# petuum/adaptdl

Hardware: AMD Instinct MI355X
Metric: goodput (samples/s x stat-eff), ResNet-18 CIFAR adaptive-BS (higher is better)
Workload: dtype bf16; 1 GPU; model=resnet18-cifar, global_batch=4096, atomic_bsz=1024, accum_steps=3, init_batch=128, max_batch=4096, parallelism=dp1

## Files before the change

adaptdl_amd/ops/hip/bindings.cpp:

```cpp

#include <torch/extension.h>
#include <ATen/hip/HIPContext.h>
#include <hip/hip_runtime.h>

#include <cmath>

#include "kernels.h"

namespace {

void check_f32(const torch::Tensor& t, const char* name) {
    TORCH_CHECK(t.is_cuda(), name, " must be a GPU tensor");
    TORCH_CHECK(t.scalar_type() == torch::kFloat32, name, " must be float32");
    TORCH_CHECK(t.is_contiguous(), name, " must be contiguous");
}

void check_out(const torch::Tensor& out) {
    TORCH_CHECK(out.is_cuda(), "out must be a GPU tensor");
    TORCH_CHECK(out.scalar_type() == torch::kFloat64, "out must be float64");
}

hipStream_t stream() {
    return at::hip::getCurrentHIPStream().stream();
}
// ... 124 lines not shown
    float bias1 = (float)(1.0 - std::pow(beta1, (double)step));
    float bias2 = (float)(1.0 - std::pow(beta2, (double)step));
    launch_fused_adamw(p.data_ptr<float>(), g.data_ptr<float>(),
                       m.data_ptr<float>(), v.data_ptr<float>(), n,
                       (float)lr, (float)beta1, (float)beta2, (float)eps,
                       (float)weight_decay, bias1, bias2, (int)adam_mode,
                       stream());
}

StatDtype check_lp_pair(const torch::Tensor& p, const torch::Tensor& g) {
    const StatDtype dtype = check_stat_in(p, "p");
    check_stat_in(g, "g");
    TORCH_CHECK(dtype != STAT_F32,
                "p must be bfloat16 or float16 (float32 parameters take "
                "fused_sgd / fused_adamw)");
    TORCH_CHECK(g.scalar_type() == p.scalar_type(), "p/g dtype mismatch");
    TORCH_CHECK(g.numel() == p.numel(), "p/g size mismatch");
    return dtype;
}

void check_f32_n(const torch::Tensor& t, long n, const char* name) {
    check_f32(t, name);
    TORCH_CHECK(t.numel() == n, name, " size mismatch");
}

void fused_sgd_mw(torch::Tensor p, torch::Tensor g, torch::Tensor w,
                  torch::Tensor m, double lr, double momentum,
                  double weight_decay, double dampening, bool nesterov) {
    const StatDtype dtype = check_lp_pair(p, g);
    long n = p.numel();
    check_f32_n(w, n, "master");
    bool has_m = momentum != 0.0;
    if (has_m) check_f32_n(m, n, "momentum_buf");
    if (n == 0) return;
    launch_fused_sgd_mw(dtype, p.data_ptr(), g.data_ptr(),
                        w.data_ptr<float>(),
                        has_m ? m.data_ptr<float>() : nullptr, n, (float)lr,
                        (float)momentum, (float)weight_decay,
                        (float)dampening, (int)nesterov, (int)has_m,
                        stream());
}

void fused_adamw_mw(torch::Tensor p, torch::Tensor g, torch::Tensor w,
                    torch::Tensor m, torch::Tensor v, double lr,
                    double beta1, double beta2, double eps,
                    double weight_decay, long step, bool adam_mode) {
    const StatDtype dtype = check_lp_pair(p, g);
    long n = p.numel();
    check_f32_n(w, n, "master");
    check_f32_n(m, n, "m"); check_f32_n(v, n, "v");
    if (n == 0) return;
    float bias1 = (float)(1.0 - std::pow(beta1, (double)step));
    float bias2 = (float)(1.0 - std::pow(beta2, (double)step));
    launch_fused_adamw_mw(dtype, p.data_ptr(), g.data_ptr(),
                          w.data_ptr<float>(), m.data_ptr<float>(),
                          v.data_ptr<float>(), n, (float)lr, (float)beta1,
                          (float)beta2, (float)eps, (float)weight_decay,
                          bias1, bias2, (int)adam_mode, stream());
}


void check_bn_x(const torch::Tensor& t, const char* name) {
    TORCH_CHECK(t.is_cuda(), name, " must be a GPU tensor");
    TORCH_CHECK(t.scalar_type() == torch::kBFloat16, name,
                " must be bfloat16");
    TORCH_CHECK(t.dim() == 4, name, " must be 4-D NCHW-shaped");
    TORCH_CHECK(t.is_contiguous(at::MemoryFormat::ChannelsLast), name,
                " must be channels_last");
}

void check_vecf(const torch::Tensor& t, long n, const char* name) {
    TORCH_CHECK(t.is_cuda() && t.scalar_type() == torch::kFloat32 &&
                t.is_contiguous() && t.numel() == n,
                name, " must be a contiguous fp32 GPU tensor of size ", n);
}

long bn_ws_rows(long m, long c) {
    TORCH_CHECK(c >= 8 && c % 8 == 0 && c / 8 <= 256,
                "bn_num_rblocks requires C % 8 == 0 and 8 <= C <= 2048, "
                "got C=", c);
    return bn_num_rblocks(m, (int)c);
}

void bn_fwd(torch::Tensor x, torch::Tensor z, torch::Tensor y,
            torch::Tensor gamma, torch::Tensor beta,
            torch::Tensor running_mean, torch::Tensor running_var,
            double momentum, double eps, bool train, bool relu,
            torch::Tensor ws, torch::Tensor sums,
            torch::Tensor save_mean, torch::Tensor save_rstd,
            torch::Tensor scale, torch::Tensor shift) {
    check_bn_x(x, "x"); check_bn_x(y, "y");
    const unsigned short* zp = nullptr;
    if (z.defined() && z.numel() > 0) {
        check_bn_x(z, "z");
        TORCH_CHECK(z.sizes() == x.sizes(), "residual shape mismatch");
        zp = (const unsigned short*)z.data_ptr();
    }
    const long c = x.size(1);
    const long m = x.numel() / c;
    TORCH_CHECK(c % 8 == 0 && c / 8 <= 256,
                "bn_fwd requires C % 8 == 0 and C <= 2048, got C=", c);
    check_vecf(gamma, c, "gamma"); check_vecf(beta, c, "beta");
    if (train)
        check_vecf(ws, 2 * c * bn_num_rblocks(m, (int)c), "ws");
    check_vecf(sums, 2 * c, "sums");
    check_vecf(save_mean, c, "save_mean");
    check_vecf(save_rstd, c, "save_rstd");
    check_vecf(scale, c, "scale"); check_vecf(shift, c, "shift");
    float* rm = nullptr;
    float* rv = nullptr;
    if (running_mean.defined() && running_mean.numel() > 0) {
        check_vecf(running_mean, c, "running_mean");
        check_vecf(running_var, c, "running_var");
        rm = running_mean.data_ptr<float>();
        rv = running_var.data_ptr<float>();
    } else {
        TORCH_CHECK(train, "eval-mode bn_fwd requires running statistics");
    }
    launch_bn_fwd((const unsigned short*)x.data_ptr(), zp,
                  (unsigned short*)y.data_ptr(), m, (int)c,
                  gamma.data_ptr<float>(), beta.data_ptr<float>(), rm, rv,
                  (float)momentum, (float)eps, (int)train, (int)relu,
                  train ? ws.data_ptr<float>() : nullptr,
                  sums.data_ptr<float>(), save_mean.data_ptr<float>(),
                  save_rstd.data_ptr<float>(), scale.data_ptr<float>(),
                  shift.data_ptr<float>(), stream());
}

void bn_bwd(torch::Tensor x, torch::Tensor z, torch::Tensor dy,
            torch::Tensor dx, torch::Tensor dz,
            torch::Tensor gamma, torch::Tensor save_mean,
            torch::Tensor save_rstd, torch::Tensor scale,
            torch::Tensor shift, bool train, bool relu, torch::Tensor ws,
            torch::Tensor sums, torch::Tensor dgamma, torch::Tensor dbeta,
            torch::Tensor pqr) {
    check_bn_x(x, "x"); check_bn_x(dy, "dy"); check_bn_x(dx, "dx");
    const unsigned short* zp = nullptr;
    unsigned short* dzp = nullptr;
    if (z.defined() && z.numel() > 0) {
        check_bn_x(z, "z"); check_bn_x(dz, "dz");
        TORCH_CHECK(z.sizes() == x.sizes(), "residual shape mismatch");
        zp = (const unsigned short*)z.data_ptr();
        dzp = (unsigned short*)dz.data_ptr();
    }
    const long c = x.size(1);
    const long m = x.numel() / c;
    check_vecf(gamma, c, "gamma");
    check_vecf(save_mean, c, "save_mean");
    check_vecf(save_rstd, c, "save_rstd");
    check_vecf(scale, c, "scale"); check_vecf(shift, c, "shift");
    check_vecf(ws, 2 * c * bn_num_rblocks(m, (int)c), "ws");
    check_vecf(sums, 2 * c, "sums");
    check_vecf(dgamma, c, "dgamma"); check_vecf(dbeta, c, "dbeta");
    check_vecf(pqr, 3 * c, "pqr");
    launch_bn_bwd((const unsigned short*)x.data_ptr(), zp,
                  (const unsigned short*)dy.data_ptr(),
                  (unsigned short*)dx.data_ptr(), dzp, m, (int)c,
                  gamma.data_ptr<float>(), save_mean.data_ptr<float>(),
                  save_rstd.data_ptr<float>(), scale.data_ptr<float>(),
                  shift.data_ptr<float>(), (int)train, (int)relu,
                  ws.data_ptr<float>(), sums.data_ptr<float>(),
                  dgamma.data_ptr<float>(), dbeta.data_ptr<float>(),
                  pqr.data_ptr<float>(), stream());
}


bool conv_wrw_ok(long N, long H, long W, long C, long K) {
    return conv3x3_wrw_supported((int)H, (int)W, (int)C, (int)K) != 0;
}

long conv_wrw_nsplit(long N, long H, long W, long C, long K) {
    return conv3x3_wrw_nsplit((int)N, (int)H, (int)W, (int)C, (int)K);
}

void conv_wrw(torch::Tensor x, torch::Tensor dy, torch::Tensor ws,
              torch::Tensor dw) {
    check_bn_x(x, "x"); check_bn_x(dy, "dy");
    const long N = x.size(0), C = x.size(1), H = x.size(2), W = x.size(3);
    const long K = dy.size(1);
    TORCH_CHECK(dy.size(0) == N && dy.size(2) == H && dy.size(3) == W,
                "dy shape mismatch");
    TORCH_CHECK(conv_wrw_ok(N, H, W, C, K), "unsupported wrw shape");
    TORCH_CHECK(dw.is_cuda() && dw.scalar_type() == torch::kFloat32 &&
                dw.is_contiguous(at::MemoryFormat::ChannelsLast) &&
                dw.size(0) == K && dw.size(1) == C && dw.size(2) == 3 &&
                dw.size(3) == 3, "dw must be (K,C,3,3) channels_last f32");
    const long nsplit = conv_wrw_nsplit(N, H, W, C, K);
    check_vecf(ws, nsplit * K * 9 * C, "ws");
    launch_conv3x3_wrw((const unsigned short*)x.data_ptr(),
                       (const unsigned short*)dy.data_ptr(),
                       ws.data_ptr<float>(), dw.data_ptr<float>(),
                       (int)N, (int)H, (int)W, (int)C, (int)K, stream());
}

bool conv_mm_ok(long N, long H, long W, long C, long K) {
    return conv3x3_mm_supported((int)H, (int)W, (int)C, (int)K) != 0;
}

void conv_mm(torch::Tensor x, torch::Tensor w, torch::Tensor y) {
    check_bn_x(x, "x"); check_bn_x(y, "y");
    const long N = x.size(0), C = x.size(1), H = x.size(2),
        Wd = x.size(3);
    const long K = y.size(1);
    TORCH_CHECK(y.size(0) == N && y.size(2) == H && y.size(3) == Wd,
                "y shape mismatch");
    TORCH_CHECK(w.is_cuda() && w.scalar_type() == torch::kBFloat16 &&
                w.is_contiguous(at::MemoryFormat::ChannelsLast) &&
                w.size(0) == K && w.size(1) == C && w.size(2) == 3 &&
                w.size(3) == 3, "w must be (K,C,3,3) channels_last bf16");
    TORCH_CHECK(conv_mm_ok(N, H, Wd, C, K), "unsupported conv_mm shape");
    launch_conv3x3_mm((const unsigned short*)x.data_ptr(),
                      (const unsigned short*)w.data_ptr(),
                      (unsigned short*)y.data_ptr(),
                      (int)N, (int)H, (int)Wd, (int)C, (int)K, stream());
}

bool conv_s2_bwd_ok(long N, long Ho, long Wo, long K, long C) {
    (void)N;
    return conv3x3_s2_bwd_supported((int)Ho, (int)Wo, (int)K, (int)C)
        != 0;
}

void conv_s2_bwd(torch::Tensor dy, torch::Tensor wt, torch::Tensor dx) {
    check_bn_x(dy, "dy"); check_bn_x(dx, "dx");
    const long N = dy.size(0), K = dy.size(1), Ho = dy.size(2),
        Wo = dy.size(3);
    const long C = dx.size(1);
    TORCH_CHECK(dx.size(0) == N && dx.size(2) == 2 * Ho &&
                dx.size(3) == 2 * Wo, "dx shape mismatch");
    TORCH_CHECK(wt.is_cuda() && wt.scalar_type() == torch::kBFloat16 &&
                wt.is_contiguous() && wt.size(0) == C &&
                wt.size(1) == 3 && wt.size(2) == 3 && wt.size(3) == K,
                "wt must be (C,3,3,K) contiguous bf16");
    TORCH_CHECK(conv_s2_bwd_ok(N, Ho, Wo, K, C),
                "unsupported s2 bwd-data shape");
    launch_conv3x3_s2_bwd((const unsigned short*)dy.data_ptr(),
                          (const unsigned short*)wt.data_ptr(),
                          (unsigned short*)dx.data_ptr(),
                          (int)N, (int)Ho, (int)Wo, (int)K, (int)C,
                          stream());
}

bool conv_s2_fwd_ok(long N, long H, long W, long C, long K) {
    (void)N;
    return conv3x3_s2_fwd_supported((int)H, (int)W, (int)C, (int)K) != 0;
}
// ... 130 lines not shown
```

adaptdl_amd/ops/hip/bn_kernels.hip:

```cpp

#include <hip/hip_runtime.h>
#include <hip/hip_bf16.h>

#include "kernels.h"

#define WAVE 64
#define BLOCK 256
#define MAX_RBLOCKS 1024
#define MAX_BLOCKS 2048
#define VEC 8

typedef unsigned short ushort_t;

union Vec8 {
    float4 f4;
    ushort_t u[VEC];
};

__device__ __forceinline__ float b2f(ushort_t h) {
    union { float f; unsigned u; } c;
    c.u = ((unsigned)h) << 16;
    return c.f;
}

__device__ __forceinline__ ushort_t f2b(float f) {
    __hip_bfloat16 h = __float2bfloat16(f);
    return *reinterpret_cast<ushort_t*>(&h);
}

__device__ __forceinline__ void rg_tree_reduce(
        float (&s)[VEC], float* lds, int slots, int rpb, int rg) {
    int p2 = 1;
    while (p2 * 2 <= rpb) p2 *= 2;
    #pragma unroll
    for (int k = 0; k < VEC; ++k) lds[threadIdx.x * VEC + k] = s[k];
    __syncthreads();
    if (rg < p2 && rg + p2 < rpb) {
        #pragma unroll
        for (int k = 0; k < VEC; ++k)
            s[k] += lds[(threadIdx.x + p2 * slots) * VEC + k];
    }
    for (int r = p2 / 2; r > 0; r >>= 1) {
        if (rg < p2) {
            #pragma unroll
            for (int k = 0; k < VEC; ++k) lds[threadIdx.x * VEC + k] = s[k];
        }
        __syncthreads();
        if (rg < r) {
            #pragma unroll
            for (int k = 0; k < VEC; ++k)
                s[k] += lds[(threadIdx.x + r * slots) * VEC + k];
        }
        __syncthreads();
    }
}

extern "C" __global__ __launch_bounds__(BLOCK) void k_bn_fwd_reduce(
        const ushort_t* __restrict__ x, long m, int c, int nb,
        float* __restrict__ ws) {
    const int slots = c / VEC;
    const int rpb = BLOCK / slots > 0 ? BLOCK / slots : 1;
    const int slot = threadIdx.x % slots;
    const int rg = threadIdx.x / slots;
    __shared__ float lds[BLOCK * VEC];

    float s[VEC], s2[VEC];
    #pragma unroll
    for (int k = 0; k < VEC; ++k) { s[k] = 0.f; s2[k] = 0.f; }

    if (rg < rpb) {
        const ushort_t* base = x + (size_t)slot * VEC;
        for (long row = (long)blockIdx.x * rpb + rg; row < m;
                row += (long)gridDim.x * rpb) {
            Vec8 v;
            v.f4 = *reinterpret_cast<const float4*>(base + (size_t)row * c);
            #pragma unroll
            for (int k = 0; k < VEC; ++k) {
                float f = b2f(v.u[k]);
                s[k] += f;
                s2[k] = fmaf(f, f, s2[k]);
            }
        }
    }
    rg_tree_reduce(s, lds, slots, rpb, rg);
    if (rg == 0) {
        #pragma unroll
        for (int k = 0; k < VEC; ++k)
            ws[(size_t)(slot * VEC + k) * nb + blockIdx.x] = s[k];
    }
    __syncthreads();
    rg_tree_reduce(s2, lds, slots, rpb, rg);
    if (rg == 0) {
        #pragma unroll
        for (int k = 0; k < VEC; ++k)
            ws[(size_t)(c + slot * VEC + k) * nb + blockIdx.x] = s2[k];
    }
}

extern "C" __global__ __launch_bounds__(BLOCK) void k_bn_reduce_ws(
        const float* __restrict__ ws, int nb, float* __restrict__ out) {
    __shared__ float lds[BLOCK];
    const float* row = ws + (size_t)blockIdx.x * nb;
    float s = 0.f;
    for (int i = threadIdx.x; i < nb; i += BLOCK) s += row[i];
    #pragma unroll
    for (int off = WAVE / 2; off > 0; off >>= 1)
        s += __shfl_down(s, off, WAVE);
    const int lane = threadIdx.x & (WAVE - 1);
    const int wid = threadIdx.x / WAVE;
    if (lane == 0) lds[wid] = s;
    __syncthreads();
    if (threadIdx.x == 0) {
        float t = 0.f;
        #pragma unroll
        for (int i = 0; i < BLOCK / WAVE; ++i) t += lds[i];
        out[blockIdx.x] = t;
    }
}

extern "C" __global__ void k_bn_fwd_finalize(
        const float* __restrict__ sums, long m, int c,
        const float* __restrict__ gamma, const float* __restrict__ beta,
        float* __restrict__ running_mean, float* __restrict__ running_var,
        float momentum, float eps,
        float* __restrict__ save_mean, float* __restrict__ save_rstd,
        float* __restrict__ scale, float* __restrict__ shift) {
    int i = blockIdx.x * blockDim.x + threadIdx.x;
    if (i >= c) return;
    float inv_m = 1.0f / (float)m;
    float mean = sums[i] * inv_m;
    float var = sums[c + i] * inv_m - mean * mean;
    var = var > 0.f ? var : 0.f;
    float rstd = rsqrtf(var + eps);
    save_mean[i] = mean;
    save_rstd[i] = rstd;
    float sc = gamma[i] * rstd;
    scale[i] = sc;
    shift[i] = beta[i] - mean * sc;
    if (running_mean != nullptr) {
        float unbiased = m > 1 ? var * (float)m / (float)(m - 1) : var;
        running_mean[i] += momentum * (mean - running_mean[i]);
        running_var[i] += momentum * (unbiased - running_var[i]);
    }
}

extern "C" __global__ void k_bn_eval_finalize(
        int c, const float* __restrict__ gamma,
        const float* __restrict__ beta,
        const float* __restrict__ running_mean,
        const float* __restrict__ running_var, float eps,
        float* __restrict__ save_mean, float* __restrict__ save_rstd,
        float* __restrict__ scale, float* __restrict__ shift) {
    int i = blockIdx.x * blockDim.x + threadIdx.x;
    if (i >= c) return;
    float mean = running_mean[i];
    float rstd = rsqrtf(running_var[i] + eps);
    save_mean[i] = mean;
    save_rstd[i] = rstd;
    float sc = gamma[i] * rstd;
    scale[i] = sc;
    shift[i] = beta[i] - mean * sc;
}

extern "C" __global__ __launch_bounds__(BLOCK) void k_bn_fwd_apply(
        const ushort_t* __restrict__ x, const ushort_t* __restrict__ z,
        ushort_t* __restrict__ y, long m, int c,
        const float* __restrict__ scale,
        const float* __restrict__ shift, int relu) {
    const int slots = c / VEC;
    const int rpb = BLOCK / slots > 0 ? BLOCK / slots : 1;
    const int slot = threadIdx.x % slots;
    const int rg = threadIdx.x / slots;
    if (rg >= rpb) return;
    float sc[VEC], sh[VEC];
    #pragma unroll
    for (int k = 0; k < VEC; ++k) {
        sc[k] = scale[slot * VEC + k];
        sh[k] = shift[slot * VEC + k];
    }
    const ushort_t* xb = x + (size_t)slot * VEC;
    const ushort_t* zb = z ? z + (size_t)slot * VEC : nullptr;
    ushort_t* yb = y + (size_t)slot * VEC;
    for (long row = (long)blockIdx.x * rpb + rg; row < m;
            row += (long)gridDim.x * rpb) {
        Vec8 in, vz, out;
        in.f4 = *reinterpret_cast<const float4*>(xb + (size_t)row * c);
        if (zb)
            vz.f4 = *reinterpret_cast<const float4*>(zb + (size_t)row * c);
        #pragma unroll
        for (int k = 0; k < VEC; ++k) {
            float f = fmaf(b2f(in.u[k]), sc[k], sh[k]);
            if (zb) f += b2f(vz.u[k]);
            if (relu) f = f > 0.f ? f : 0.f;
            out.u[k] = f2b(f);
        }
        *reinterpret_cast<float4*>(yb + (size_t)row * c) = out.f4;
    }
}

extern "C" __global__ __launch_bounds__(BLOCK) void k_bn_bwd_reduce(
        const ushort_t* __restrict__ x, const ushort_t* __restrict__ z,
        const ushort_t* __restrict__ dy,
        long m, int c, int nb, const float* __restrict__ mean,
        const float* __restrict__ rstd, const float* __restrict__ scale,
        const float* __restrict__ shift, int relu,
        float* __restrict__ ws) {
    const int slots = c / VEC;
    const int rpb = BLOCK / slots > 0 ? BLOCK / slots : 1;
    const int slot = threadIdx.x % slots;
    const int rg = threadIdx.x / slots;
    __shared__ float lds[BLOCK * VEC];

    float sg[VEC], sgx[VEC];
    float mn[VEC], rs[VEC], sc[VEC], sh[VEC];
    #pragma unroll
    for (int k = 0; k < VEC; ++k) {
        sg[k] = 0.f; sgx[k] = 0.f;
        mn[k] = mean[slot * VEC + k];
        rs[k] = rstd[slot * VEC + k];
        sc[k] = scale[slot * VEC + k];
        sh[k] = shift[slot * VEC + k];
    }
    if (rg < rpb) {
        const ushort_t* xb = x + (size_t)slot * VEC;
        const ushort_t* zb = z ? z + (size_t)slot * VEC : nullptr;
        const ushort_t* db = dy + (size_t)slot * VEC;
        for (long row = (long)blockIdx.x * rpb + rg; row < m;
                row += (long)gridDim.x * rpb) {
            Vec8 vx, vz, vd;
            vx.f4 = *reinterpret_cast<const float4*>(xb + (size_t)row * c);
            if (zb)
                vz.f4 = *reinterpret_cast<const float4*>(
                    zb + (size_t)row * c);
            vd.f4 = *reinterpret_cast<const float4*>(db + (size_t)row * c);
            #pragma unroll
            for (int k = 0; k < VEC; ++k) {
                float fx = b2f(vx.u[k]);
                float g = b2f(vd.u[k]);
                if (relu) {
                    float pre = fmaf(fx, sc[k], sh[k]);
                    if (zb) pre += b2f(vz.u[k]);
                    if (pre <= 0.f) g = 0.f;
                }
                sg[k] += g;
                sgx[k] = fmaf(g, (fx - mn[k]) * rs[k], sgx[k]);
            }
        }
    }
    rg_tree_reduce(sg, lds, slots, rpb, rg);
    if (rg == 0) {
        #pragma unroll
        for (int k = 0; k < VEC; ++k)
            ws[(size_t)(slot * VEC + k) * nb + blockIdx.x] = sg[k];
    }
    __syncthreads();
    rg_tree_reduce(sgx, lds, slots, rpb, rg);
    if (rg == 0) {
        #pragma unroll
        for (int k = 0; k < VEC; ++k)
            ws[(size_t)(c + slot * VEC + k) * nb + blockIdx.x] = sgx[k];
    }
}

extern "C" __global__ void k_bn_bwd_finalize(
        const float* __restrict__ sums, long m, int c,
        const float* __restrict__ gamma, const float* __restrict__ mean,
        const float* __restrict__ rstd, int train,
        float* __restrict__ dgamma, float* __restrict__ dbeta,
        float* __restrict__ pqr) {
    int i = blockIdx.x * blockDim.x + threadIdx.x;
    if (i >= c) return;
    float sum_g = sums[i];
    float sum_gx = sums[c + i];
    dbeta[i] = sum_g;
    dgamma[i] = sum_gx;
    float p = gamma[i] * rstd[i];
    float q = 0.f, r = 0.f;
    if (train) {
        float inv_m = 1.0f / (float)m;
        q = p * (sum_gx * inv_m) * rstd[i];
        r = -p * (sum_g * inv_m) + q * mean[i];
    }
    pqr[i] = p;
    pqr[c + i] = q;
    pqr[2 * c + i] = r;
}

extern "C" __global__ __launch_bounds__(BLOCK) void k_bn_bwd_apply(
        const ushort_t* __restrict__ x, const ushort_t* __restrict__ z,
        const ushort_t* __restrict__ dy,
        ushort_t* __restrict__ dx, ushort_t* __restrict__ dz, long m,
        int c, const float* __restrict__ scale,
        const float* __restrict__ shift,
        const float* __restrict__ pqr, int relu) {
    const int slots = c / VEC;
    const int rpb = BLOCK / slots > 0 ? BLOCK / slots : 1;
    const int slot = threadIdx.x % slots;
    const int rg = threadIdx.x / slots;
    if (rg >= rpb) return;
    float sc[VEC], sh[VEC], cp[VEC], cq[VEC], cr[VEC];
    #pragma unroll
    for (int k = 0; k < VEC; ++k) {
        sc[k] = scale[slot * VEC + k];
        sh[k] = shift[slot * VEC + k];
        cp[k] = pqr[slot * VEC + k];
        cq[k] = pqr[c + slot * VEC + k];
        cr[k] = pqr[2 * c + slot * VEC + k];
    }
    const ushort_t* xb = x + (size_t)slot * VEC;
    const ushort_t* zb = z ? z + (size_t)slot * VEC : nullptr;
    const ushort_t* db = dy + (size_t)slot * VEC;
    ushort_t* ob = dx + (size_t)slot * VEC;
    ushort_t* zo = dz ? dz + (size_t)slot * VEC : nullptr;
    for (long row = (long)blockIdx.x * rpb + rg; row < m;
            row += (long)gridDim.x * rpb) {
        Vec8 vx, vz, vd, out, outz;
        vx.f4 = *reinterpret_cast<const float4*>(xb + (size_t)row * c);
        if (zb)
            vz.f4 = *reinterpret_cast<const float4*>(zb + (size_t)row * c);
        vd.f4 = *reinterpret_cast<const float4*>(db + (size_t)row * c);
        #pragma unroll
        for (int k = 0; k < VEC; ++k) {
            float fx = b2f(vx.u[k]);
            float g = b2f(vd.u[k]);
            if (relu) {
                float pre = fmaf(fx, sc[k], sh[k]);
                if (zb) pre += b2f(vz.u[k]);
                if (pre <= 0.f) g = 0.f;
            }
            if (zo) outz.u[k] = f2b(g);
            out.u[k] = f2b(fmaf(cp[k], g, fmaf(-cq[k], fx, cr[k])));
        }
        *reinterpret_cast<float4*>(ob + (size_t)row * c) = out.f4;
        if (zo)
            *reinterpret_cast<float4*>(zo + (size_t)row * c) = outz.f4;
    }
}


static inline unsigned bn_grid(long work_items, int per_block, long cap) {
    long blocks = (work_items + per_block - 1) / per_block;
    if (blocks > cap) blocks = cap;
    if (blocks < 1) blocks = 1;
    return (unsigned)blocks;
}

static inline int bn_rows_per_block(int c) {
    const int slots = c / VEC;
    return BLOCK / slots > 0 ? BLOCK / slots : 1;
}

extern "C" long bn_num_rblocks(long m, int c) {
    return bn_grid(m, bn_rows_per_block(c), MAX_RBLOCKS);
}

extern "C" void launch_bn_fwd(
        const ushort_t* x, const ushort_t* z, ushort_t* y, long m, int c,
        const float* gamma, const float* beta, float* running_mean,
        float* running_var, float momentum, float eps, int train, int relu,
        float* ws, float* sums, float* save_mean, float* save_rstd,
        float* scale, float* shift, hipStream_t s) {
    const int rpb = bn_rows_per_block(c);
    if (train) {
        const unsigned nb = (unsigned)bn_num_rblocks(m, c);
        hipLaunchKernelGGL(k_bn_fwd_reduce, dim3(nb), dim3(BLOCK), 0, s,
                           x, m, c, (int)nb, ws);
        hipLaunchKernelGGL(k_bn_reduce_ws, dim3(2 * c), dim3(BLOCK), 0, s,
                           ws, (int)nb, sums);
        hipLaunchKernelGGL(k_bn_fwd_finalize,
                           dim3((c + BLOCK - 1) / BLOCK), dim3(BLOCK), 0, s,
                           sums, m, c, gamma, beta, running_mean,
                           running_var, momentum, eps, save_mean, save_rstd,
                           scale, shift);
    } else {
        hipLaunchKernelGGL(k_bn_eval_finalize,
                           dim3((c + BLOCK - 1) / BLOCK), dim3(BLOCK), 0, s,
                           c, gamma, beta, running_mean, running_var, eps,
                           save_mean, save_rstd, scale, shift);
    }
    hipLaunchKernelGGL(k_bn_fwd_apply, dim3(bn_grid(m, rpb, MAX_BLOCKS)),
                       dim3(BLOCK), 0, s, x, z, y, m, c, scale, shift,
                       relu);
}

extern "C" void launch_bn_bwd(
        const ushort_t* x, const ushort_t* z, const ushort_t* dy,
        ushort_t* dx, ushort_t* dz, long m, int c,
        const float* gamma, const float* save_mean, const float* save_rstd,
        const float* scale, const float* shift, int train, int relu,
        float* ws, float* sums, float* dgamma, float* dbeta, float* pqr,
        hipStream_t s) {
    const int rpb = bn_rows_per_block(c);
    const unsigned nb = (unsigned)bn_num_rblocks(m, c);
    hipLaunchKernelGGL(k_bn_bwd_reduce, dim3(nb), dim3(BLOCK), 0, s,
                       x, z, dy, m, c, (int)nb, save_mean, save_rstd,
                       scale, shift, relu, ws);
    hipLaunchKernelGGL(k_bn_reduce_ws, dim3(2 * c), dim3(BLOCK), 0, s,
                       ws, (int)nb, sums);
    hipLaunchKernelGGL(k_bn_bwd_finalize, dim3((c + BLOCK - 1) / BLOCK),
                       dim3(BLOCK), 0, s, sums, m, c, gamma, save_mean,
                       save_rstd, train, dgamma, dbeta, pqr);
    hipLaunchKernelGGL(k_bn_bwd_apply, dim3(bn_grid(m, rpb, MAX_BLOCKS)),
                       dim3(BLOCK), 0, s, x, z, dy, dx, dz, m, c, scale,
                       shift, pqr, relu);
}
```

adaptdl_amd/ops/hip/kernels.h:

```cpp

#pragma once

#include <hip/hip_runtime_api.h>

extern "C" {

enum StatDtype { STAT_F32 = 0, STAT_BF16 = 1, STAT_FP16 = 2 };


void launch_sqsum(StatDtype dtype, const void* x, long n, double* out,
                  hipStream_t s);
void launch_scale_sqsum(StatDtype dtype, void* x, long n, float scale,
                        double* out, hipStream_t s);
void launch_sqsum_diff_update(StatDtype dtype, const void* cur, void* prev,
                              long n, double* out, hipStream_t s);
void launch_sqsum_avg(StatDtype dtype, const void* cur, const void* prev,
                      long n, double* out, hipStream_t s);
void launch_precond_sqsum(const float* g, const float* v, long n,
                          float inv_corr_sqrt, float eps, double* out,
                          hipStream_t s);
void launch_precond_sqsum_dev(const float* g, const float* v, long n,
                              const float* pc, double* out, hipStream_t s);
void launch_fused_sgd(float* p, const float* g, float* m, long n, float lr,
                      float momentum, float weight_decay, float dampening,
                      int nesterov, int has_momentum, hipStream_t s);
void launch_fused_adamw(float* p, const float* g, float* m, float* v,
                        long n, float lr, float beta1, float beta2,
                        float eps, float weight_decay, float bias1,
                        float bias2, int adam_mode, hipStream_t s);

void launch_precond_sqsum_mw(StatDtype dtype, const void* g,
                             const float* v, long n, float inv_corr_sqrt,
                             float eps, double* out, hipStream_t s);
void launch_precond_sqsum_dev_mw(StatDtype dtype, const void* g,
                                 const float* v, long n, const float* pc,
                                 double* out, hipStream_t s);
void launch_fused_sgd_mw(StatDtype dtype, void* p, const void* g,
                         float* w, float* m, long n, float lr,
                         float momentum, float weight_decay,
                         float dampening, int nesterov, int has_momentum,
                         hipStream_t s);
void launch_fused_adamw_mw(StatDtype dtype, void* p, const void* g,
                           float* w, float* m, float* v, long n, float lr,
                           float beta1, float beta2, float eps,
                           float weight_decay, float bias1, float bias2,
                           int adam_mode, hipStream_t s);


long bn_num_rblocks(long m, int c);
void launch_bn_fwd(const unsigned short* x, const unsigned short* z,
                   unsigned short* y, long m, int c, const float* gamma,
                   const float* beta, float* running_mean,
                   float* running_var, float momentum, float eps,
                   int train, int relu, float* ws, float* sums,
                   float* save_mean, float* save_rstd, float* scale,
                   float* shift, hipStream_t s);
void launch_bn_bwd(const unsigned short* x, const unsigned short* z,
                   const unsigned short* dy, unsigned short* dx,
                   unsigned short* dz, long m, int c, const float* gamma,
                   const float* save_mean, const float* save_rstd,
                   const float* scale, const float* shift, int train,
                   int relu, float* ws, float* sums, float* dgamma,
                   float* dbeta, float* pqr, hipStream_t s);


int conv3x3_wrw_params(int H, int W, int* P, int* Wp);
int conv3x3_wrw_supported(int H, int W, int C, int K);
int conv3x3_wrw_nsplit(int N, int H, int W, int C, int K);
void launch_conv3x3_wrw(const unsigned short* x, const unsigned short* dy,
                        float* ws, float* dw, int N, int H, int W, int C,
                        int K, hipStream_t s);
int conv3x3_mm_supported(int H, int W, int C, int K);
void launch_conv3x3_mm(const unsigned short* x, const unsigned short* w,
                       unsigned short* y, int N, int H, int W, int C,
                       int K, hipStream_t s);
int conv3x3_s2_fwd_supported(int H, int W, int C, int K);
void launch_conv3x3_s2_fwd(const unsigned short* x,
                           const unsigned short* w, unsigned short* y,
                           int N, int H, int W, int C, int K,
                           hipStream_t s);
int conv3x3_s2_bwd_supported(int Ho, int Wo, int K, int C);
void launch_conv3x3_s2_bwd(const unsigned short* dy,
                           const unsigned short* wt, unsigned short* dx,
                           int N, int Ho, int Wo, int K, int C,
                           hipStream_t s);
int conv3x3_s2_wrw_supported(int Ho, int Wo, int C, int K);
int conv3x3_s2_wrw_nsplit(int N, int Ho, int Wo, int C, int K);
void launch_conv3x3_s2_wrw(const unsigned short* x,
                           const unsigned short* dy, float* ws, float* dw,
                           int N, int Ho, int Wo, int C, int K,
                           hipStream_t s);
int conv3x3_s2_bwd_w8b_supported(int Ho, int Wo, int K, int C);
void launch_conv3x3_s2_bwd_w8b(const unsigned short* dy,
                               const unsigned short* wt,
                               unsigned short* dx, int N, int Ho, int K,
                               int C, hipStream_t s);

}
```

adaptdl_amd/torch/layers.py:

```python

import os

import torch
import torch.nn as nn
import torch.nn.functional as F

from adaptdl_amd import ops


def _hip_bn_ok(x):
    c = x.shape[1] if x.dim() == 4 else 0
    return (x.is_cuda and x.dtype == torch.bfloat16 and x.dim() == 4 and
            c % 8 == 0 and c // 8 <= 256 and
            x.is_contiguous(memory_format=torch.channels_last) and
            ops.has_extension())


class _FusedBNFunction(torch.autograd.Function):
    @staticmethod
    def forward(ctx, x, z, weight, bias, running_mean, running_var,
                training, momentum, eps, relu):
        ext = ops._load_extension()
        y = torch.empty_like(x)
        c = x.shape[1]
        m = x.numel() // c
        opt = dict(dtype=torch.float32, device=x.device)
        ws = torch.empty(2 * c * ext.bn_num_rblocks(m, c), **opt) \
            if training else torch.empty(0, **opt)
        sums = torch.empty(2 * c, **opt)
        save_mean = torch.empty(c, **opt)
        save_rstd = torch.empty(c, **opt)
        scale = torch.empty(c, **opt)
        shift = torch.empty(c, **opt)
        none = torch.empty(0, **opt)
        znone = torch.empty(0, dtype=x.dtype, device=x.device)
        ext.bn_fwd(x, z if z is not None else znone, y, weight, bias,
                   running_mean if running_mean is not None else none,
                   running_var if running_var is not None else none,
                   float(momentum), float(eps), bool(training), bool(relu),
                   ws, sums, save_mean, save_rstd, scale, shift)
        ctx.save_for_backward(x, z if z is not None else znone, weight,
                              save_mean, save_rstd, scale, shift)
        ctx.bn_train = bool(training)
        ctx.bn_relu = bool(relu)
        ctx.bn_has_z = z is not None
        return y

    @staticmethod
    def backward(ctx, dy):
        ext = ops._load_extension()
        x, z, weight, save_mean, save_rstd, scale, shift = \
            ctx.saved_tensors
        dy = dy.contiguous(memory_format=torch.channels_last)
        dx = torch.empty_like(x)
        dz = torch.empty_like(x) if ctx.bn_has_z else \
            torch.empty(0, dtype=x.dtype, device=x.device)
        c = x.shape[1]
        m = x.numel() // c
        opt = dict(dtype=torch.float32, device=x.device)
        ws = torch.empty(2 * c * ext.bn_num_rblocks(m, c), **opt)
        sums = torch.empty(2 * c, **opt)
        dgamma = torch.empty(c, **opt)
        dbeta = torch.empty(c, **opt)
        pqr = torch.empty(3 * c, **opt)
        ext.bn_bwd(x, z, dy, dx, dz, weight, save_mean, save_rstd, scale,
                   shift, ctx.bn_train, ctx.bn_relu, ws, sums, dgamma,
                   dbeta, pqr)
        return (dx, dz if ctx.bn_has_z else None, dgamma, dbeta) + \
            (None,) * 6


class FusedBatchNormAct2d(nn.BatchNorm2d):

    def __init__(self, num_features, eps=1e-5, momentum=0.1, affine=True,
                 track_running_stats=True, relu=False):
        super().__init__(num_features, eps=eps, momentum=momentum,
                         affine=affine,
                         track_running_stats=track_running_stats)
        self.relu = relu

    def forward(self, x, residual=None):
        use_batch_stats = self.training or not self.track_running_stats
        if _hip_bn_ok(x) and self.affine and \
                (residual is None or
                 (residual.dtype == x.dtype and residual.is_contiguous(
                     memory_format=torch.channels_last))):
            if self.training and self.track_running_stats and \
                    self.num_batches_tracked is not None:
                self.num_batches_tracked.add_(1)
            momentum = self.momentum if self.momentum is not None else 0.0
            return _FusedBNFunction.apply(
                x, residual, self.weight, self.bias, self.running_mean,
                self.running_var, use_batch_stats, momentum, self.eps,
                self.relu)
        y = super().forward(x)
        if residual is not None:
            y = y + residual
        return F.relu(y) if self.relu else y


class _FusedConvFunction(torch.autograd.Function):

    @staticmethod
    def forward(ctx, x, weight, wb, stride, padding, dilation, groups):
        ext = ops._load_extension()
        n, c, h, w = x.shape
        k = wb.shape[0]
        if os.getenv("ADAPTDL_EXPERIMENTAL_CONV_MM") == "1" \
                and ext.conv_mm_ok(n, h, w, c, k):
            y = torch.empty(n, k, h, w, dtype=x.dtype, device=x.device) \
                .contiguous(memory_format=torch.channels_last)
            ext.conv_mm(x, wb, y)
        else:
            y = torch.nn.functional.conv2d(x, wb, None, stride, padding,
                                           dilation, groups)
        ctx.save_for_backward(x, wb)
        ctx.conv_args = (stride, padding, dilation, groups)
        return y

    @staticmethod
    def backward(ctx, dy):
        ext = ops._load_extension()
        x, wb = ctx.saved_tensors
        stride, padding, dilation, groups = ctx.conv_args
        dy = dy.contiguous(memory_format=torch.channels_last)
        dx = None
        if ctx.needs_input_grad[0]:
            n, c, h, w = x.shape
            k = wb.shape[0]
            if os.getenv("ADAPTDL_EXPERIMENTAL_CONV_MM") == "1" \
                    and ext.conv_mm_ok(n, h, w, k, c):
                wt = wb.flip(2, 3).permute(1, 0, 2, 3) \
                    .contiguous(memory_format=torch.channels_last)
                dx = torch.empty_like(x)
                ext.conv_mm(dy, wt, dx)
            else:
                dx = torch.ops.aten.convolution_backward(
                    dy, x, wb, None, stride, padding, dilation, False,
                    [0, 0], groups, [True, False, False])[0]
        n, c, h, w = x.shape
        k = dy.shape[1]
        nsplit = ext.conv_wrw_nsplit(n, h, w, c, k)
        ws = torch.empty(nsplit * k * 9 * c, dtype=torch.float32,
                         device=x.device)
        dw = torch.empty(k, c, 3, 3, dtype=torch.float32,
                         device=x.device) \
            .contiguous(memory_format=torch.channels_last)
        ext.conv_wrw(x, dy, ws, dw)
        return dx, dw, None, None, None, None, None


class _S2ConvFunction(torch.autograd.Function):

    @staticmethod
    def forward(ctx, x, weight, stride, padding, dilation, groups):
        wb = weight.detach().to(torch.bfloat16) \
            .contiguous(memory_format=torch.channels_last)
        y = torch.nn.functional.conv2d(x, wb, None, stride, padding,
                                       dilation, groups)
        ctx.save_for_backward(x, wb)
        ctx.conv_args = (stride, padding, dilation, groups)
        return y

    @staticmethod
    def backward(ctx, dy):
        ext = ops._load_extension()
        x, wb = ctx.saved_tensors
        stride, padding, dilation, groups = ctx.conv_args
        dy = dy.contiguous(memory_format=torch.channels_last)
        dx = dw = None
        if ctx.needs_input_grad[0]:
            wt = wb.permute(1, 2, 3, 0).contiguous()
            dx = torch.empty_like(x)
            n2, k2, ho2, wo2 = dy.shape
            if os.getenv("ADAPTDL_S2_W8B") == "1" and wo2 == 8 \
                    and ext.conv_s2_bwd_w8b_ok(n2, ho2, wo2, k2,
                                               x.shape[1]):
# ... 130 lines not shown
```

Baseline: 22210 goodput-samples/s.

## Fuse BN workspace reduce into finalize tail and save ReLU mask for residual BN

Merges the separate workspace row-reduction and finalize kernels into one per-channel tail kernel in both BN forward and backward, removing a launch and the intermediate sums buffer. The num_batches_tracked increment moves into that kernel, dropping a separate PyTorch add op. For ReLU+residual BN, the forward pass writes a 1-bit-per-element mask so backward can skip re-reading the residual and recomputing the pre-activation. This costs an extra uint8 write in forward, and the residual is no longer kept for backward.

Result: faster. 22880 goodput-samples/s, median of 6 (+3.0%).

```diff
diff --git a/adaptdl_amd/ops/hip/bindings.cpp b/adaptdl_amd/ops/hip/bindings.cpp
--- a/adaptdl_amd/ops/hip/bindings.cpp
+++ b/adaptdl_amd/ops/hip/bindings.cpp
@@ -230,14 +230,25 @@
     return bn_num_rblocks(m, (int)c);
 }
 
+unsigned char* bn_mask_ptr(const torch::Tensor& mask, long m, long c) {
+    if (!mask.defined() || mask.numel() == 0) return nullptr;
+    TORCH_CHECK(mask.is_cuda() && mask.scalar_type() == torch::kUInt8 &&
+                mask.is_contiguous() && mask.numel() == m * (c / 8),
+                "mask must be a contiguous uint8 GPU tensor of size ",
+                m * (c / 8));
+    return mask.data_ptr<unsigned char>();
+}
+
 void bn_fwd(torch::Tensor x, torch::Tensor z, torch::Tensor y,
             torch::Tensor gamma, torch::Tensor beta,
             torch::Tensor running_mean, torch::Tensor running_var,
             double momentum, double eps, bool train, bool relu,
-            torch::Tensor ws, torch::Tensor sums,
+            torch::Tensor ws,
             torch::Tensor save_mean, torch::Tensor save_rstd,
-            torch::Tensor scale, torch::Tensor shift) {
+            torch::Tensor scale, torch::Tensor shift,
+            torch::Tensor mask, torch::Tensor num_batches_tracked) {
     check_bn_x(x, "x"); check_bn_x(y, "y");
+    TORCH_CHECK(y.sizes() == x.sizes(), "output shape mismatch");
     const unsigned short* zp = nullptr;
     if (z.defined() && z.numel() > 0) {
         check_bn_x(z, "z");
@@ -251,7 +262,6 @@
     check_vecf(gamma, c, "gamma"); check_vecf(beta, c, "beta");
     if (train)
         check_vecf(ws, 2 * c * bn_num_rblocks(m, (int)c), "ws");
-    check_vecf(sums, 2 * c, "sums");
     check_vecf(save_mean, c, "save_mean");
     check_vecf(save_rstd, c, "save_rstd");
     check_vecf(scale, c, "scale"); check_vecf(shift, c, "shift");
@@ -265,14 +275,25 @@
     } else {
         TORCH_CHECK(train, "eval-mode bn_fwd requires running statistics");
     }
+    unsigned char* mp = bn_mask_ptr(mask, m, c);
+    TORCH_CHECK(mp == nullptr || (relu && zp != nullptr),
+                "a ReLU mask is stored only with relu and a residual");
+    long long* nbt = nullptr;
+    if (num_batches_tracked.defined() && num_batches_tracked.numel() > 0) {
+        TORCH_CHECK(num_batches_tracked.is_cuda() &&
+                    num_batches_tracked.scalar_type() == torch::kInt64 &&
+                    num_batches_tracked.numel() == 1,
+                    "num_batches_tracked must be an int64 GPU scalar");
+        nbt = (long long*)num_batches_tracked.data_ptr<int64_t>();
+    }
     launch_bn_fwd((const unsigned short*)x.data_ptr(), zp,
                   (unsigned short*)y.data_ptr(), m, (int)c,
                   gamma.data_ptr<float>(), beta.data_ptr<float>(), rm, rv,
                   (float)momentum, (float)eps, (int)train, (int)relu,
                   train ? ws.data_ptr<float>() : nullptr,
-                  sums.data_ptr<float>(), save_mean.data_ptr<float>(),
+                  save_mean.data_ptr<float>(),
                   save_rstd.data_ptr<float>(), scale.data_ptr<float>(),
-                  shift.data_ptr<float>(), stream());
+                  shift.data_ptr<float>(), mp, nbt, stream());
 }
 
 void bn_bwd(torch::Tensor x, torch::Tensor z, torch::Tensor dy,
@@ -280,25 +301,36 @@
             torch::Tensor gamma, torch::Tensor save_mean,
             torch::Tensor save_rstd, torch::Tensor scale,
             torch::Tensor shift, bool train, bool relu, torch::Tensor ws,
-            torch::Tensor sums, torch::Tensor dgamma, torch::Tensor dbeta,
-            torch::Tensor pqr) {
+            torch::Tensor dgamma, torch::Tensor dbeta,
+            torch::Tensor pqr, torch::Tensor mask) {
     check_bn_x(x, "x"); check_bn_x(dy, "dy"); check_bn_x(dx, "dx");
+    TORCH_CHECK(dy.sizes() == x.sizes() && dx.sizes() == x.sizes(),
+                "gradient shape mismatch");
+    const long c = x.size(1);
+    const long m = x.numel() / c;
+    TORCH_CHECK(c % 8 == 0 && c / 8 <= 256,
+                "bn_bwd requires C % 8 == 0 and C <= 2048, got C=", c);
     const unsigned short* zp = nullptr;
     unsigned short* dzp = nullptr;
+    const unsigned char* mp = bn_mask_ptr(mask, m, c);
     if (z.defined() && z.numel() > 0) {
-        check_bn_x(z, "z"); check_bn_x(dz, "dz");
+        check_bn_x(z, "z");
         TORCH_CHECK(z.sizes() == x.sizes(), "residual shape mismatch");
         zp = (const unsigned short*)z.data_ptr();
+    }
+    if (dz.defined() && dz.numel() > 0) {
+        check_bn_x(dz, "dz");
+        TORCH_CHECK(dz.sizes() == x.sizes(), "residual shape mismatch");
+        TORCH_CHECK(zp != nullptr || mp != nullptr,
+                    "dz requires the residual or its saved ReLU mask");
         dzp = (unsigned short*)dz.data_ptr();
     }
-    const long c = x.size(1);
-    const long m = x.numel() / c;
+    TORCH_CHECK(mp == nullptr || relu, "a ReLU mask requires relu");
     check_vecf(gamma, c, "gamma");
     check_vecf(save_mean, c, "save_mean");
     check_vecf(save_rstd, c, "save_rstd");
     check_vecf(scale, c, "scale"); check_vecf(shift, c, "shift");
     check_vecf(ws, 2 * c * bn_num_rblocks(m, (int)c), "ws");
-    check_vecf(sums, 2 * c, "sums");
     check_vecf(dgamma, c, "dgamma"); check_vecf(dbeta, c, "dbeta");
     check_vecf(pqr, 3 * c, "pqr");
     launch_bn_bwd((const unsigned short*)x.data_ptr(), zp,
@@ -307,9 +339,9 @@
                   gamma.data_ptr<float>(), save_mean.data_ptr<float>(),
                   save_rstd.data_ptr<float>(), scale.data_ptr<float>(),
                   shift.data_ptr<float>(), (int)train, (int)relu,
-                  ws.data_ptr<float>(), sums.data_ptr<float>(),
+                  ws.data_ptr<float>(),
                   dgamma.data_ptr<float>(), dbeta.data_ptr<float>(),
-                  pqr.data_ptr<float>(), stream());
+                  pqr.data_ptr<float>(), mp, stream());
 }
 
 
diff --git a/adaptdl_amd/ops/hip/bn_kernels.hip b/adaptdl_amd/ops/hip/bn_kernels.hip
--- a/adaptdl_amd/ops/hip/bn_kernels.hip
+++ b/adaptdl_amd/ops/hip/bn_kernels.hip
@@ -97,50 +97,81 @@
     }
 }
 
-extern "C" __global__ __launch_bounds__(BLOCK) void k_bn_reduce_ws(
-        const float* __restrict__ ws, int nb, float* __restrict__ out) {
-    __shared__ float lds[BLOCK];
-    const float* row = ws + (size_t)blockIdx.x * nb;
-    float s = 0.f;
-    for (int i = threadIdx.x; i < nb; i += BLOCK) s += row[i];
-    #pragma unroll
-    for (int off = WAVE / 2; off > 0; off >>= 1)
-        s += __shfl_down(s, off, WAVE);
+#define WS_TRIPS (MAX_RBLOCKS / BLOCK)
+static_assert(WS_TRIPS * BLOCK == MAX_RBLOCKS, "row-sum trips cover a row");
+
+__device__ __forceinline__ void ws_row_pair_sum(
+        const float* __restrict__ ws, int nb, int c, int ch, float* lds,
+        float& t0, float& t1) {
+    const float* row0 = ws + (size_t)ch * nb;
+    const float* row1 = ws + (size_t)(c + ch) * nb;
+    float a[WS_TRIPS], b[WS_TRIPS];
+    #pragma unroll
+    for (int j = 0; j < WS_TRIPS; ++j) {
+        const int i = min((int)threadIdx.x + j * BLOCK, nb - 1);
+        a[j] = row0[i];
+        b[j] = row1[i];
+    }
+    float s0 = 0.f, s1 = 0.f;
+    #pragma unroll
+    for (int j = 0; j < WS_TRIPS; ++j) {
+        if ((int)threadIdx.x + j * BLOCK < nb) { s0 += a[j]; s1 += b[j]; }
+    }
+    #pragma unroll
+    for (int off = WAVE / 2; off > 0; off >>= 1) {
+        s0 += __shfl_down(s0, off, WAVE);
+        s1 += __shfl_down(s1, off, WAVE);
+    }
     const int lane = threadIdx.x & (WAVE - 1);
     const int wid = threadIdx.x / WAVE;
-    if (lane == 0) lds[wid] = s;
+    if (lane == 0) {
+        lds[wid] = s0;
+        lds[BLOCK / WAVE + wid] = s1;
+    }
     __syncthreads();
+    t0 = 0.f; t1 = 0.f;
     if (threadIdx.x == 0) {
-        float t = 0.f;
-        #pragma unroll
-        for (int i = 0; i < BLOCK / WAVE; ++i) t += lds[i];
-        out[blockIdx.x] = t;
-    }
-}
-
-extern "C" __global__ void k_bn_fwd_finalize(
-        const float* __restrict__ sums, long m, int c,
+        #pragma unroll
+        for (int i = 0; i < BLOCK / WAVE; ++i) t0 += lds[i];
+        #pragma unroll
+        for (int i = 0; i < BLOCK / WAVE; ++i) t1 += lds[BLOCK / WAVE + i];
+    }
+}
+
+extern "C" __global__ __launch_bounds__(BLOCK) void k_bn_fwd_tail(
+        const float* __restrict__ ws, int nb, long m, int c,
         const float* __restrict__ gamma, const float* __restrict__ beta,
         float* __restrict__ running_mean, float* __restrict__ running_var,
         float momentum, float eps,
         float* __restrict__ save_mean, float* __restrict__ save_rstd,
-        float* __restrict__ scale, float* __restrict__ shift) {
-    int i = blockIdx.x * blockDim.x + threadIdx.x;
-    if (i >= c) return;
-    float inv_m = 1.0f / (float)m;
-    float mean = sums[i] * inv_m;
-    float var = sums[c + i] * inv_m - mean * mean;
-    var = var > 0.f ? var : 0.f;
-    float rstd = rsqrtf(var + eps);
-    save_mean[i] = mean;
-    save_rstd[i] = rstd;
-    float sc = gamma[i] * rstd;
-    scale[i] = sc;
-    shift[i] = beta[i] - mean * sc;
-    if (running_mean != nullptr) {
-        float unbiased = m > 1 ? var * (float)m / (float)(m - 1) : var;
-        running_mean[i] += momentum * (mean - running_mean[i]);
-        running_var[i] += momentum * (unbiased - running_var[i]);
+        float* __restrict__ scale, float* __restrict__ shift,
+        long long* __restrict__ num_batches_tracked) {
+    __shared__ float lds[2 * BLOCK / WAVE];
+    const int i = blockIdx.x;
+    const float g = gamma[i], b = beta[i];
+    const float rm = running_mean ? running_mean[i] : 0.f;
+    const float rv = running_mean ? running_var[i] : 0.f;
+    float sum, sumsq;
+    ws_row_pair_sum(ws, nb, c, i, lds, sum, sumsq);
+    if (threadIdx.x == 0) {
+        #pragma clang fp contract(off)
+        float inv_m = 1.0f / (float)m;
+        float mean = sum * inv_m;
+        float var = sumsq * inv_m - mean * mean;
+        var = var > 0.f ? var : 0.f;
+        float rstd = rsqrtf(var + eps);
+        save_mean[i] = mean;
+        save_rstd[i] = rstd;
+        float sc = g * rstd;
+        scale[i] = sc;
+        shift[i] = fmaf(-mean, sc, b);
+        if (running_mean != nullptr) {
+            float unbiased = m > 1 ? var * (float)m / (float)(m - 1) : var;
+            running_mean[i] = fmaf(momentum, mean - rm, rm);
+            running_var[i] = fmaf(momentum, unbiased - rv, rv);
+        }
+        if (i == 0 && num_batches_tracked != nullptr)
+            *num_batches_tracked += 1;
     }
 }
 
@@ -166,7 +197,8 @@
         const ushort_t* __restrict__ x, const ushort_t* __restrict__ z,
         ushort_t* __restrict__ y, long m, int c,
         const float* __restrict__ scale,
-        const float* __restrict__ shift, int relu) {
+        const float* __restrict__ shift, int relu,
+        unsigned char* __restrict__ mask) {
     const int slots = c / VEC;
     const int rpb = BLOCK / slots > 0 ? BLOCK / slots : 1;
     const int slot = threadIdx.x % slots;
@@ -187,14 +219,17 @@
         in.f4 = *reinterpret_cast<const float4*>(xb + (size_t)row * c);
         if (zb)
             vz.f4 = *reinterpret_cast<const float4*>(zb + (size_t)row * c);
+        unsigned bits = 0;
         #pragma unroll
         for (int k = 0; k < VEC; ++k) {
             float f = fmaf(b2f(in.u[k]), sc[k], sh[k]);
             if (zb) f += b2f(vz.u[k]);
+            if (f > 0.f) bits |= 1u << k;
             if (relu) f = f > 0.f ? f : 0.f;
             out.u[k] = f2b(f);
         }
         *reinterpret_cast<float4*>(yb + (size_t)row * c) = out.f4;
+        if (mask) mask[(size_t)row * slots + slot] = (unsigned char)bits;
     }
 }
 
@@ -204,7 +239,7 @@
         long m, int c, int nb, const float* __restrict__ mean,
         const float* __restrict__ rstd, const float* __restrict__ scale,
         const float* __restrict__ shift, int relu,
-        float* __restrict__ ws) {
+        const unsigned char* __restrict__ mask, float* __restrict__ ws) {
     const int slots = c / VEC;
     const int rpb = BLOCK / slots > 0 ? BLOCK / slots : 1;
     const int slot = threadIdx.x % slots;
@@ -233,11 +268,15 @@
                 vz.f4 = *reinterpret_cast<const float4*>(
                     zb + (size_t)row * c);
             vd.f4 = *reinterpret_cast<const float4*>(db + (size_t)row * c);
+            unsigned bits = 0;
+            if (mask) bits = mask[(size_t)row * slots + slot];
             #pragma unroll
             for (int k = 0; k < VEC; ++k) {
                 float fx = b2f(vx.u[k]);
                 float g = b2f(vd.u[k]);
-                if (relu) {
+                if (mask) {
+                    if (!((bits >> k) & 1u)) g = 0.f;
+                } else if (relu) {
                     float pre = fmaf(fx, sc[k], sh[k]);
                     if (zb) pre += b2f(vz.u[k]);
                     if (pre <= 0.f) g = 0.f;
@@ -262,28 +301,32 @@
     }
 }
 
-extern "C" __global__ void k_bn_bwd_finalize(
-        const float* __restrict__ sums, long m, int c,
+extern "C" __global__ __launch_bounds__(BLOCK) void k_bn_bwd_tail(
+        const float* __restrict__ ws, int nb, long m, int c,
         const float* __restrict__ gamma, const float* __restrict__ mean,
         const float* __restrict__ rstd, int train,
         float* __restrict__ dgamma, float* __restrict__ dbeta,
         float* __restrict__ pqr) {
-    int i = blockIdx.x * blockDim.x + threadIdx.x;
-    if (i >= c) return;
-    float sum_g = sums[i];
-    float sum_gx = sums[c + i];
-    dbeta[i] = sum_g;
-    dgamma[i] = sum_gx;
-    float p = gamma[i] * rstd[i];
-    float q = 0.f, r = 0.f;
-    if (train) {
-        float inv_m = 1.0f / (float)m;
-        q = p * (sum_gx * inv_m) * rstd[i];
-        r = -p * (sum_g * inv_m) + q * mean[i];
-    }
-    pqr[i] = p;
-    pqr[c + i] = q;
-    pqr[2 * c + i] = r;
+    __shared__ float lds[2 * BLOCK / WAVE];
+    const int i = blockIdx.x;
+    const float g = gamma[i], rs = rstd[i], mn = mean[i];
+    float sum_g, sum_gx;
+    ws_row_pair_sum(ws, nb, c, i, lds, sum_g, sum_gx);
+    if (threadIdx.x == 0) {
+        #pragma clang fp contract(off)
+        dbeta[i] = sum_g;
+        dgamma[i] = sum_gx;
+        float p = g * rs;
+        float q = 0.f, r = 0.f;
+        if (train) {
+            float inv_m = 1.0f / (float)m;
+            q = p * (sum_gx * inv_m) * rs;
+            r = -p * (sum_g * inv_m) + q * mn;
+        }
+        pqr[i] = p;
+        pqr[c + i] = q;
+        pqr[2 * c + i] = r;
+    }
 }
 
 extern "C" __global__ __launch_bounds__(BLOCK) void k_bn_bwd_apply(
@@ -292,7 +335,8 @@
         ushort_t* __restrict__ dx, ushort_t* __restrict__ dz, long m,
         int c, const float* __restrict__ scale,
         const float* __restrict__ shift,
-        const float* __restrict__ pqr, int relu) {
+        const float* __restrict__ pqr, int relu,
+        const unsigned char* __restrict__ mask) {
     const int slots = c / VEC;
     const int rpb = BLOCK / slots > 0 ? BLOCK / slots : 1;
     const int slot = threadIdx.x % slots;
@@ -319,11 +363,15 @@
         if (zb)
             vz.f4 = *reinterpret_cast<const float4*>(zb + (size_t)row * c);
         vd.f4 = *reinterpret_cast<const float4*>(db + (size_t)row * c);
+        unsigned bits = 0;
+        if (mask) bits = mask[(size_t)row * slots + slot];
         #pragma unroll
         for (int k = 0; k < VEC; ++k) {
             float fx = b2f(vx.u[k]);
             float g = b2f(vd.u[k]);
-            if (relu) {
+            if (mask) {
+                if (!((bits >> k) & 1u)) g = 0.f;
+            } else if (relu) {
                 float pre = fmaf(fx, sc[k], sh[k]);
                 if (zb) pre += b2f(vz.u[k]);
                 if (pre <= 0.f) g = 0.f;
@@ -358,29 +406,28 @@
         const ushort_t* x, const ushort_t* z, ushort_t* y, long m, int c,
         const float* gamma, const float* beta, float* running_mean,
         float* running_var, float momentum, float eps, int train, int relu,
-        float* ws, float* sums, float* save_mean, float* save_rstd,
-        float* scale, float* shift, hipStream_t s) {
+        float* ws, float* save_mean, float* save_rstd, float* scale,
+        float* shift, unsigned char* mask, long long* num_batches_tracked,
+        hipStream_t s) {
     const int rpb = bn_rows_per_block(c);
     if (train) {
         const unsigned nb = (unsigned)bn_num_rblocks(m, c);
         hipLaunchKernelGGL(k_bn_fwd_reduce, dim3(nb), dim3(BLOCK), 0, s,
                            x, m, c, (int)nb, ws);
-        hipLaunchKernelGGL(k_bn_reduce_ws, dim3(2 * c), dim3(BLOCK), 0, s,
-                           ws, (int)nb, sums);
-        hipLaunchKernelGGL(k_bn_fwd_finalize,
-                           dim3((c + BLOCK - 1) / BLOCK), dim3(BLOCK), 0, s,
-                           sums, m, c, gamma, beta, running_mean,
+        hipLaunchKernelGGL(k_bn_fwd_tail, dim3(c), dim3(BLOCK), 0, s,
+                           ws, (int)nb, m, c, gamma, beta, running_mean,
                            running_var, momentum, eps, save_mean, save_rstd,
-                           scale, shift);
+                           scale, shift, num_batches_tracked);
     } else {
         hipLaunchKernelGGL(k_bn_eval_finalize,
                            dim3((c + BLOCK - 1) / BLOCK), dim3(BLOCK), 0, s,
                            c, gamma, beta, running_mean, running_var, eps,
                            save_mean, save_rstd, scale, shift);
     }
+    if (!(relu && z)) mask = nullptr;
     hipLaunchKernelGGL(k_bn_fwd_apply, dim3(bn_grid(m, rpb, MAX_BLOCKS)),
                        dim3(BLOCK), 0, s, x, z, y, m, c, scale, shift,
-                       relu);
+                       relu, mask);
 }
 
 extern "C" void launch_bn_bwd(
@@ -388,19 +435,18 @@
         ushort_t* dx, ushort_t* dz, long m, int c,
         const float* gamma, const float* save_mean, const float* save_rstd,
         const float* scale, const float* shift, int train, int relu,
-        float* ws, float* sums, float* dgamma, float* dbeta, float* pqr,
-        hipStream_t s) {
+        float* ws, float* dgamma, float* dbeta, float* pqr,
+        const unsigned char* mask, hipStream_t s) {
     const int rpb = bn_rows_per_block(c);
     const unsigned nb = (unsigned)bn_num_rblocks(m, c);
+    if (!relu) mask = nullptr;
     hipLaunchKernelGGL(k_bn_bwd_reduce, dim3(nb), dim3(BLOCK), 0, s,
                        x, z, dy, m, c, (int)nb, save_mean, save_rstd,
-                       scale, shift, relu, ws);
-    hipLaunchKernelGGL(k_bn_reduce_ws, dim3(2 * c), dim3(BLOCK), 0, s,
-                       ws, (int)nb, sums);
-    hipLaunchKernelGGL(k_bn_bwd_finalize, dim3((c + BLOCK - 1) / BLOCK),
-                       dim3(BLOCK), 0, s, sums, m, c, gamma, save_mean,
-                       save_rstd, train, dgamma, dbeta, pqr);
+                       scale, shift, relu, mask, ws);
+    hipLaunchKernelGGL(k_bn_bwd_tail, dim3(c), dim3(BLOCK), 0, s,
+                       ws, (int)nb, m, c, gamma, save_mean, save_rstd,
+                       train, dgamma, dbeta, pqr);
     hipLaunchKernelGGL(k_bn_bwd_apply, dim3(bn_grid(m, rpb, MAX_BLOCKS)),
                        dim3(BLOCK), 0, s, x, z, dy, dx, dz, m, c, scale,
-                       shift, pqr, relu);
-}
+                       shift, pqr, relu, mask);
+}
diff --git a/adaptdl_amd/ops/hip/kernels.h b/adaptdl_amd/ops/hip/kernels.h
--- a/adaptdl_amd/ops/hip/kernels.h
+++ b/adaptdl_amd/ops/hip/kernels.h
@@ -52,16 +52,17 @@
                    unsigned short* y, long m, int c, const float* gamma,
                    const float* beta, float* running_mean,
                    float* running_var, float momentum, float eps,
-                   int train, int relu, float* ws, float* sums,
-                   float* save_mean, float* save_rstd, float* scale,
-                   float* shift, hipStream_t s);
+                   int train, int relu, float* ws, float* save_mean,
+                   float* save_rstd, float* scale, float* shift,
+                   unsigned char* mask, long long* num_batches_tracked,
+                   hipStream_t s);
 void launch_bn_bwd(const unsigned short* x, const unsigned short* z,
                    const unsigned short* dy, unsigned short* dx,
                    unsigned short* dz, long m, int c, const float* gamma,
                    const float* save_mean, const float* save_rstd,
                    const float* scale, const float* shift, int train,
-                   int relu, float* ws, float* sums, float* dgamma,
-                   float* dbeta, float* pqr, hipStream_t s);
+                   int relu, float* ws, float* dgamma, float* dbeta,
+                   float* pqr, const unsigned char* mask, hipStream_t s);
 
 
 int conv3x3_wrw_params(int H, int W, int* P, int* Wp);
diff --git a/adaptdl_amd/torch/layers.py b/adaptdl_amd/torch/layers.py
--- a/adaptdl_amd/torch/layers.py
+++ b/adaptdl_amd/torch/layers.py
@@ -19,7 +19,8 @@
 class _FusedBNFunction(torch.autograd.Function):
     @staticmethod
     def forward(ctx, x, z, weight, bias, running_mean, running_var,
-                training, momentum, eps, relu):
+                training, momentum, eps, relu, num_batches_tracked=None,
+                save_mask=False):
         ext = ops._load_extension()
         y = torch.empty_like(x)
         c = x.shape[1]
@@ -27,20 +28,25 @@
         opt = dict(dtype=torch.float32, device=x.device)
         ws = torch.empty(2 * c * ext.bn_num_rblocks(m, c), **opt) \
             if training else torch.empty(0, **opt)
-        sums = torch.empty(2 * c, **opt)
         save_mean = torch.empty(c, **opt)
         save_rstd = torch.empty(c, **opt)
         scale = torch.empty(c, **opt)
         shift = torch.empty(c, **opt)
         none = torch.empty(0, **opt)
         znone = torch.empty(0, dtype=x.dtype, device=x.device)
+        use_mask = bool(relu) and z is not None and bool(save_mask)
+        mask = torch.empty(m * (c // 8) if use_mask else 0,
+                           dtype=torch.uint8, device=x.device)
+        nbt = num_batches_tracked if num_batches_tracked is not None \
+            else torch.empty(0, dtype=torch.int64, device=x.device)
         ext.bn_fwd(x, z if z is not None else znone, y, weight, bias,
                    running_mean if running_mean is not None else none,
                    running_var if running_var is not None else none,
                    float(momentum), float(eps), bool(training), bool(relu),
-                   ws, sums, save_mean, save_rstd, scale, shift)
-        ctx.save_for_backward(x, z if z is not None else znone, weight,
-                              save_mean, save_rstd, scale, shift)
+                   ws, save_mean, save_rstd, scale, shift, mask, nbt)
+        ctx.save_for_backward(
+            x, z if z is not None and not use_mask else znone, mask,
+            weight, save_mean, save_rstd, scale, shift)
         ctx.bn_train = bool(training)
         ctx.bn_relu = bool(relu)
         ctx.bn_has_z = z is not None
@@ -49,7 +55,7 @@
     @staticmethod
     def backward(ctx, dy):
         ext = ops._load_extension()
-        x, z, weight, save_mean, save_rstd, scale, shift = \
+        x, z, mask, weight, save_mean, save_rstd, scale, shift = \
             ctx.saved_tensors
         dy = dy.contiguous(memory_format=torch.channels_last)
         dx = torch.empty_like(x)
@@ -59,15 +65,14 @@
         m = x.numel() // c
         opt = dict(dtype=torch.float32, device=x.device)
         ws = torch.empty(2 * c * ext.bn_num_rblocks(m, c), **opt)
-        sums = torch.empty(2 * c, **opt)
         dgamma = torch.empty(c, **opt)
         dbeta = torch.empty(c, **opt)
         pqr = torch.empty(3 * c, **opt)
         ext.bn_bwd(x, z, dy, dx, dz, weight, save_mean, save_rstd, scale,
-                   shift, ctx.bn_train, ctx.bn_relu, ws, sums, dgamma,
-                   dbeta, pqr)
+                   shift, ctx.bn_train, ctx.bn_relu, ws, dgamma, dbeta,
+                   pqr, mask)
         return (dx, dz if ctx.bn_has_z else None, dgamma, dbeta) + \
-            (None,) * 6
+            (None,) * 8
 
 
 class FusedBatchNormAct2d(nn.BatchNorm2d):
@@ -85,14 +90,16 @@
                 (residual is None or
                  (residual.dtype == x.dtype and residual.is_contiguous(
                      memory_format=torch.channels_last))):
-            if self.training and self.track_running_stats and \
-                    self.num_batches_tracked is not None:
-                self.num_batches_tracked.add_(1)
+            nbt = self.num_batches_tracked if self.training and \
+                self.track_running_stats else None
             momentum = self.momentum if self.momentum is not None else 0.0
+            needs_bwd = torch.is_grad_enabled() and any(
+                t is not None and t.requires_grad
+                for t in (x, residual, self.weight, self.bias))
             return _FusedBNFunction.apply(
                 x, residual, self.weight, self.bias, self.running_mean,
                 self.running_var, use_batch_stats, momentum, self.eps,
-                self.relu)
+                self.relu, nbt, needs_bwd)
         y = super().forward(x)
         if residual is not None:
             y = y + residual
```
